# traveller59/spconv

Hardware: NVIDIA H100
Metric: active-voxels/sec fwd+bwd SubMConv3d 3^3 C=64 (higher is better)
Workload: dtype fp16

## Files before the change

### spconv_b200/csrc/common.cuh

```cuda
#pragma once
#include <cuda_runtime.h>
#include <cuda_fp16.h>
#include <cuda_bf16.h>
#include <stdint.h>
#include <stdio.h>
#include <string.h>
#include <stdarg.h>
#include <type_traits>

#include "../../include/spconv_b200.h"

namespace spx {

void set_error(const char *fmt, ...);
void count_launch(int n = 1);
void set_family(int f);
int sm_count();
int current_device();

struct RuntimeCfg {
    int force_simt = 0, force_tc = 0;
    bool tf32_dgrad_fma = false;
    bool tf32_wgrad_fma = false;
};
RuntimeCfg &runtime_cfg();

bool func_configured(const void *fn, int dev);

#define SPX_CHECK_CUDA(expr)                                                              \
    do {                                                                                  \
        cudaError_t _e = (expr);                                                          \
        if (_e != cudaSuccess) {                                                          \
            (void)cudaGetLastError();                                                     \
            spx::set_error("%s failed: %s (%s:%d)", #expr, cudaGetErrorString(_e),        \
                           __FILE__, __LINE__);                                           \
            return 1;                                                                     \
        }                                                                                 \
    } while (0)

#define SPX_CHECK_LAUNCH(name)                                                            \
    do {                                                                                  \
        cudaError_t _e = cudaGetLastError();                                              \
        if (_e != cudaSuccess) {                                                          \
            spx::set_error("launch of %s failed: %s (%s:%d)", name,                       \
                           cudaGetErrorString(_e), __FILE__, __LINE__);                   \
            return 1;                                                                     \
        }                                                                                 \
        spx::count_launch();                                                              \
    } while (0)

#define SPX_REQUIRE(cond, ...)                                                            \
    do {                                                                                  \
        if (!(cond)) {                                                                    \
            spx::set_error(__VA_ARGS__);                                                  \
            return 2;                                                                     \
        }                                                                                 \
    } while (0)

static inline size_t align_up(size_t x, size_t a) { return (x + a - 1) / a * a; }
static inline int64_t div_up64(int64_t a, int64_t b) { return (a + b - 1) / b; }

static inline bool aligned16(const void *p) { return ((uintptr_t)p & 15u) == 0; }

#define SPX_REQUIRE_ALIGNED16(ptr, who)                                                   \
    SPX_REQUIRE(spx::aligned16(ptr), "%s: %s must be 16-byte aligned (got %p)", who, #ptr, \
                (const void *)(ptr))

struct WorkspaceCarver {
    char *base;
    size_t off = 0, cap;
    WorkspaceCarver(void *p, size_t bytes) : base((char *)p), cap(bytes) {}
    template <typename T> T *take(size_t n) {
        off = align_up(off, 256);
        T *r = (T *)(base + off);
        off += n * sizeof(T);
        return r;
    }
    bool ok() const { return off <= cap; }
};

__host__ __device__ static inline int dtype_bytes(int dt) {
    switch (dt) {
        case SPX_F32: return 4;
        case SPX_F16: return 2;
        case SPX_BF16: return 2;
        case SPX_I8: return 1;
    }
    return 0;
}

#ifdef __CUDACC__

template <typename T> __device__ __forceinline__ float to_float(T v);
template <> __device__ __forceinline__ float to_float<float>(float v) { return v; }
template <> __device__ __forceinline__ float to_float<__half>(__half v) { return __half2float(v); }
template <> __device__ __forceinline__ float to_float<__nv_bfloat16>(__nv_bfloat16 v) { return __bfloat162float(v); }
template <> __device__ __forceinline__ float to_float<int8_t>(int8_t v) { return (float)v; }

template <typename T> __device__ __forceinline__ T from_float(float v);
template <> __device__ __forceinline__ float from_float<float>(float v) { return v; }
template <> __device__ __forceinline__ __half from_float<__half>(float v) { return __float2half_rn(v); }
template <> __device__ __forceinline__ __nv_bfloat16 from_float<__nv_bfloat16>(float v) { return __float2bfloat16_rn(v); }

__device__ __forceinline__ float apply_act(float v, int act, float alpha) {
    switch (act) {
        case SPX_ACT_RELU: return v > 0.f ? v : 0.f;
        case SPX_ACT_SIGMOID: return 1.f / (1.f + __expf(-v));
        case SPX_ACT_LEAKY_RELU: return v >= 0.f ? v : v * alpha;
        default: return v;
    }
}

__device__ __forceinline__ uint32_t smem_u32(const void *p) {
    return (uint32_t)__cvta_generic_to_shared(p);
}

__device__ __forceinline__ void mbar_init(uint64_t *bar, uint32_t count) {
    asm volatile("mbarrier.init.shared::cta.b64 [%0], %1;" ::"r"(smem_u32(bar)), "r"(count) : "memory");
}
__device__ __forceinline__ void mbar_fence_init() {
    asm volatile("fence.mbarrier_init.release.cluster;" ::: "memory");
}
__device__ __forceinline__ void mbar_arrive(uint64_t *bar) {
    asm volatile("{\n\t.reg .b64 st;\n\tmbarrier.arrive.shared::cta.b64 st, [%0];\n\t}" ::"r"(smem_u32(bar)) : "memory");
}
__device__ __forceinline__ void mbar_arrive_expect_tx(uint64_t *bar, uint32_t bytes) {
    asm volatile("{\n\t.reg .b64 st;\n\tmbarrier.arrive.expect_tx.shared::cta.b64 st, [%0], %1;\n\t}" ::"r"(smem_u32(bar)), "r"(bytes) : "memory");
}
__device__ __forceinline__ bool mbar_try_wait(uint64_t *bar, uint32_t parity) {
    uint32_t ok;
    asm volatile(
        "{\n\t.reg .pred p;\n\t"
        "mbarrier.try_wait.parity.shared::cta.b64 p, [%1], %2;\n\t"
        "selp.u32 %0, 1, 0, p;\n\t}"
        : "=r"(ok) : "r"(smem_u32(bar)), "r"(parity) : "memory");
    return ok != 0;
}
__device__ __forceinline__ void mbar_wait(uint64_t *bar, uint32_t parity) {
    if (mbar_try_wait(bar, parity)) return;
    const long long t0 = clock64();
    uint32_t spins = 0;
    while (!mbar_try_wait(bar, parity)) {
        if ((++spins & 0x3FFFu) == 0u && clock64() - t0 > 4000000000ll) {
            printf("spconv_b200: mbarrier wait timed out (block %d thread %d bar 0x%x parity %u)\n",
                   (int)blockIdx.x, (int)threadIdx.x, smem_u32(bar), parity);
            __trap();
        }
    }
}
__device__ __forceinline__ void mbar_wait_silent(uint64_t *bar, uint32_t parity) {
    if (mbar_try_wait(bar, parity)) return;
    const long long t0 = clock64();
    uint32_t spins = 0;
    while (!mbar_try_wait(bar, parity)) {
        if ((++spins & 0x3FFFu) == 0u && clock64() - t0 > 4000000000ll) __trap();
    }
}
__device__ __forceinline__ void cp_async_mbar_arrive_noinc(uint64_t *bar) {
    asm volatile("cp.async.mbarrier.arrive.noinc.shared::cta.b64 [%0];" ::"r"(smem_u32(bar)) : "memory");
}

__device__ __forceinline__ void cp_async_16(uint32_t dst_smem, const void *src, uint32_t src_bytes) {
    asm volatile("cp.async.cg.shared.global [%0], [%1], 16, %2;" ::"r"(dst_smem), "l"(src), "r"(src_bytes) : "memory");
}
__device__ __forceinline__ void cp_async_commit() { asm volatile("cp.async.commit_group;" ::: "memory"); }
template <int N> __device__ __forceinline__ void cp_async_wait() {
    asm volatile("cp.async.wait_group %0;" ::"n"(N) : "memory");
}

__device__ __forceinline__ void fence_proxy_async_smem() {
    asm volatile("fence.proxy.async.shared::cta;" ::: "memory");
}

__device__ __forceinline__ void tma_load_2d(uint32_t dst_smem, const void *tmap, uint64_t *bar,
                                            int32_t c0, int32_t c1) {
    asm volatile(
        "cp.async.bulk.tensor.2d.shared::cta.global.tile.mbarrier::complete_tx::bytes [%0], [%1, {%3, %4}], [%2];"
        ::"r"(dst_smem), "l"(tmap), "r"(smem_u32(bar)), "r"(c0), "r"(c1) : "memory");
}
__device__ __forceinline__ void bulk_copy_g2s(uint32_t dst_smem, const void *src, uint32_t bytes, uint64_t *bar) {
    asm volatile("cp.async.bulk.shared::cluster.global.mbarrier::complete_tx::bytes [%0], [%1], %2, [%3];"
                 ::"r"(dst_smem), "l"(src), "r"(bytes), "r"(smem_u32(bar)) : "memory");
}
__device__ __forceinline__ void tma_prefetch_desc(const void *tmap) {
    asm volatile("prefetch.tensormap [%0];" ::"l"(tmap) : "memory");
}

enum MmaKind { KIND_F16 = 0, KIND_TF32 = 1, KIND_I8 = 2 };

__device__ __forceinline__ void wgmma_fence() { asm volatile("wgmma.fence.sync.aligned;" ::: "memory"); }
__device__ __forceinline__ void wgmma_commit() { asm volatile("wgmma.commit_group.sync.aligned;" ::: "memory"); }
template <int N> __device__ __forceinline__ void wgmma_wait() {
    asm volatile("wgmma.wait_group.sync.aligned %0;" ::"n"(N) : "memory");
}
template <typename T, int R> __device__ __forceinline__ void fence_regs(T (&d)[R]) {
#pragma unroll
    for (int i = 0; i < R; ++i) {
        if constexpr (sizeof(T) == 4 && std::is_floating_point<T>::value) asm volatile("" : "+f"(d[i])::"memory");
        else asm volatile("" : "+r"(d[i])::"memory");
    }
}

__host__ __device__ __forceinline__ uint64_t gmma_desc_hi(uint32_t lbo_bytes, uint32_t sbo_bytes, uint32_t swizzle_bytes) {
    const uint64_t layout = swizzle_bytes == 128 ? 1ull : (swizzle_bytes == 64 ? 2ull : 3ull);
    return ((uint64_t)((lbo_bytes >> 4) & 0x3FFF) << 16) | ((uint64_t)((sbo_bytes >> 4) & 0x3FFF) << 32) | (layout << 62);
}

__device__ __forceinline__ uint32_t swizzle_offset(uint32_t off, uint32_t swizzle_bytes) {
    uint32_t bits = swizzle_bytes == 128 ? 7u : (swizzle_bytes == 64 ? 3u : 1u);
    return off ^ (((off >> 7) & bits) << 4);
}

#endif

}
```

### spconv_b200/csrc/gemm_tc.cu

```cuda
#include "gemm.cuh"
#include "wgmma.cuh"
#include <cuda.h>
#include <atomic>
#include <mutex>
#include <stdlib.h>

namespace spx {

constexpr int TC_TILE_M = 128;
constexpr int TC_CONS_WARPS = 8;
constexpr int TC_PROD_WARPS = 2;
constexpr int TC_PROD_THREADS = TC_PROD_WARPS * 32;
constexpr int TC_TMA_WARP = TC_CONS_WARPS + TC_PROD_WARPS;
constexpr int TC_SCHED_WARP = TC_TMA_WARP + 1;
constexpr int TC_THREADS = 3 * 128;
constexpr int TC_INFO_DEPTH = 4;
constexpr int TC_INFO_READERS = TC_PROD_WARPS + TC_CONS_WARPS + 1;
constexpr int TC_MAX_STAGES = 8;
constexpr int TC_SMEM_BUDGET = 200 * 1024;

struct TcParams {
    const uint8_t *x;
    int xb;
    int span_b, b_subtiles, b_sub_bytes, b_bytes, b_mn_major, b_kstep16_mn;
    int b_transposed;
    const float *w;
    int c_in, c_out;
    int w_inner_elems;
    int span_b_elems;
    int n;
    int ab_bf16;
    int stages, a_stage_bytes, stage_bytes, idx_bytes;
    int64_t rows;
    const int32_t *tile_table;
    const int32_t *sched_rec;
    int *sched_state;
    const int32_t *argsort;
    int kv, words, reverse;
    void *y;
    int out_dtype;
    int epi_mode;
    const void *bias;
    int act; float alpha;
    const float *scale, *bias_f32;
    const int8_t *output_add;
    float output_add_scale;
};

struct BitIter {
    uint32_t m0, m1, m2, m3;
    __device__ __forceinline__ BitIter(const uint32_t (&t)[4]) : m0(t[0]), m1(t[1]), m2(t[2]), m3(t[3]) {}
    __device__ __forceinline__ int next() {
        if (m0) { int b = __ffs(m0) - 1; m0 &= m0 - 1; return b; }
        if (m1) { int b = __ffs(m1) - 1; m1 &= m1 - 1; return 32 + b; }
        if (m2) { int b = __ffs(m2) - 1; m2 &= m2 - 1; return 64 + b; }
        if (m3) { int b = __ffs(m3) - 1; m3 &= m3 - 1; return 96 + b; }
        return -1;
    }
};

template <int OUT>
__device__ __forceinline__ void store2(uint8_t *dst, float a, float b) {
    if constexpr (OUT == SPX_F32) {
        *reinterpret_cast<float2 *>(dst) = make_float2(a, b);
    } else if constexpr (OUT == SPX_F16) {
        *reinterpret_cast<__half2 *>(dst) = __floats2half2_rn(a, b);
    } else if constexpr (OUT == SPX_BF16) {
        *reinterpret_cast<__nv_bfloat162 *>(dst) = __floats2bfloat162_rn(a, b);
    } else {
        const int qa = (int)fminf(fmaxf(rintf(a), -128.f), 127.f), qb = (int)fminf(fmaxf(rintf(b), -128.f), 127.f);
        *reinterpret_cast<uint16_t *>(dst) = (uint16_t)((uint32_t)(uint8_t)(int8_t)qa | ((uint32_t)(uint8_t)(int8_t)qb << 8));
    }
}

template <int OUT> struct OutElem { static constexpr int bytes = OUT == SPX_F32 ? 4 : (OUT == SPX_I8 ? 1 : 2); };

template <int OUT>
__device__ __forceinline__ float load_bias(const void *bias, int j) {
    if constexpr (OUT == SPX_F32) return ((const float *)bias)[j];
    else if constexpr (OUT == SPX_F16) return __half2float(((const __half *)bias)[j]);
    else return __bfloat162float(((const __nv_bfloat16 *)bias)[j]);
}

template <int OUT, bool INT8_MODE, int N, typename Acc, bool PLAIN = false>
__device__ __forceinline__ void epilogue_frag(const TcParams &p, const float *ec, const Acc (&acc)[N / 2], int64_t dst_lo,
                                              int64_t dst_hi, int lane) {
    if constexpr (!INT8_MODE && !PLAIN) {
        if (p.bias == nullptr && p.act == SPX_ACT_NONE) {
            epilogue_frag<OUT, false, N, Acc, true>(p, ec, acc, dst_lo, dst_hi, lane);
            return;
        }
    }
    constexpr int EB = OutElem<OUT>::bytes;
    const bool has_bias = !PLAIN && (INT8_MODE ? (p.bias_f32 != nullptr) : (p.bias != nullptr));
#pragma unroll
    for (int h = 0; h < 2; ++h) {
        const int64_t dst = h ? dst_hi : dst_lo;
        if (dst < 0) continue;
        uint8_t *row_ptr = (uint8_t *)p.y + dst * (int64_t)N * EB;
#pragma unroll
        for (int nb = 0; nb < N / 8; ++nb) {
            const int col = nb * 8 + 2 * (lane & 3);
            float f[2];
#pragma unroll
            for (int j = 0; j < 2; ++j) {
                const Acc v = acc[nb * 4 + 2 * h + j];
                if constexpr (!INT8_MODE) {
                    f[j] = (float)v;
                    if (has_bias) f[j] += ec[col + j];
                } else {
                    f[j] = (float)(int32_t)v * ec[col + j];
                    if (has_bias) f[j] += ec[N + col + j];
                    if (p.output_add) f[j] += (float)p.output_add[dst * (int64_t)N + col + j] * p.output_add_scale;
                }
                if (!PLAIN && p.act != SPX_ACT_NONE) f[j] = apply_act(f[j], p.act, p.alpha);
            }
            store2<OUT>(row_ptr + col * EB, f[0], f[1]);
        }
    }
}

template <int KIND, int N, typename Acc>
__device__ __forceinline__ void mma_step(Acc (&acc)[N / 2], uint64_t a, uint64_t b, int b_mn, int bf16) {
    if constexpr (KIND == KIND_F16) {
        if (bf16) {
            if (b_mn) Wgmma<N>::template bf16<0, 1>(acc, a, b, 1u);
            else Wgmma<N>::template bf16<0, 0>(acc, a, b, 1u);
        } else {
            if (b_mn) Wgmma<N>::template f16<0, 1>(acc, a, b, 1u);
            else Wgmma<N>::template f16<0, 0>(acc, a, b, 1u);
        }
    } else if constexpr (KIND == KIND_TF32) {
        Wgmma<N>::tf32(acc, a, b, 1u);
    } else {
        Wgmma<N>::s8(acc, a, b, 1u);
    }
}

template <int KIND, int CPR, int N>
__global__ void __launch_bounds__(TC_THREADS, 1)
tc_gather_gemm_kernel(const __grid_constant__ CUtensorMap tmap_w, const TcParams p) {
    using Acc = typename std::conditional<KIND == KIND_I8, int32_t, float>::type;
    constexpr int LG_CPR = CPR == 2 ? 1 : CPR == 4 ? 2 : CPR == 8 ? 3 : CPR == 16 ? 4 : 5;
    constexpr int RPI = 32 / CPR;
    constexpr int XB = CPR * 16;
    constexpr int SPAN_A = XB < 128 ? XB : 128;
    constexpr int LG_SPAN_A = SPAN_A == 128 ? 7 : (SPAN_A == 64 ? 6 : 5);
    constexpr int A_SUB_BYTES = TC_TILE_M * SPAN_A;
    constexpr int A_SUBTILES = XB / SPAN_A;
    constexpr int Q_A = SPAN_A / 32;
    constexpr int ROWS_PW = TC_TILE_M / TC_PROD_WARPS;
    constexpr int ITERS = ROWS_PW / RPI > 0 ? ROWS_PW / RPI : 1;
    static_assert(ROWS_PW * CPR >= 32, "a producer warp must cover at least one full cp.async instruction");

    extern __shared__ __align__(1024) uint8_t smem_raw[];
    const uint32_t raw_addr = smem_u32(smem_raw);
    const uint32_t pad = (1024u - (raw_addr & 1023u)) & 1023u;
    uint8_t *smem = smem_raw + pad;
    const uint32_t smem_base = raw_addr + pad;

    const uint32_t idx_off = (uint32_t)p.stages * p.stage_bytes;
    uint64_t *bars = reinterpret_cast<uint64_t *>(smem + idx_off + 2u * p.idx_bytes);
    uint64_t *full = bars;
    uint64_t *empty = bars + TC_MAX_STAGES;
    uint64_t *idx_full = bars + 2 * TC_MAX_STAGES;
    uint64_t *idx_empty = bars + 2 * TC_MAX_STAGES + 2;
    uint64_t *info_full = bars + 2 * TC_MAX_STAGES + 4;
    uint64_t *info_empty = bars + 2 * TC_MAX_STAGES + 4 + TC_INFO_DEPTH;
    int32_t *info = reinterpret_cast<int32_t *>(bars + 2 * TC_MAX_STAGES + 4 + 2 * TC_INFO_DEPTH);
    float *ec = reinterpret_cast<float *>(smem + idx_off + 2u * p.idx_bytes + 1024u);

    const int warp = threadIdx.x >> 5;
    const int lane = threadIdx.x & 31;
    const int64_t num_tiles = (p.rows + TC_TILE_M - 1) / TC_TILE_M;

    auto read_info = [&](int n, uint32_t (&tm)[4]) -> int {
        const int e = n & (TC_INFO_DEPTH - 1);
        mbar_wait_silent(&info_full[e], (uint32_t)((n / TC_INFO_DEPTH) & 1));
        const volatile int32_t *r = info + e * 8;
        const int tile = r[0];
        tm[0] = (uint32_t)r[1]; tm[1] = (uint32_t)r[2]; tm[2] = (uint32_t)r[3]; tm[3] = (uint32_t)r[4];
        __syncwarp();
        if (lane == 0) mbar_arrive(&info_empty[e]);
        return tile;
    };

    if (threadIdx.x == 0) {
        for (int s = 0; s < p.stages; ++s) {
            mbar_init(&full[s], TC_PROD_THREADS + 1);
            mbar_init(&empty[s], TC_CONS_WARPS);
        }
        for (int a = 0; a < 2; ++a) {
            mbar_init(&idx_full[a], 1);
            mbar_init(&idx_empty[a], TC_PROD_WARPS + TC_CONS_WARPS);
        }
        for (int e = 0; e < TC_INFO_DEPTH; ++e) {
            mbar_init(&info_full[e], 1);
            mbar_init(&info_empty[e], TC_INFO_READERS);
        }
        mbar_fence_init();
        tma_prefetch_desc(&tmap_w);
    }
    for (int j = threadIdx.x; j < N; j += TC_THREADS) {
        if constexpr (KIND == KIND_I8) {
            ec[j] = __ldg(p.scale + j);
            if (p.bias_f32) ec[N + j] = __ldg(p.bias_f32 + j);
        } else if (p.bias) {
            if constexpr (KIND == KIND_TF32) ec[j] = load_bias<SPX_F32>(p.bias, j);
            else ec[j] = p.out_dtype == SPX_F16 ? load_bias<SPX_F16>(p.bias, j) : load_bias<SPX_BF16>(p.bias, j);
        }
    }
    __syncthreads();

    if (warp >= TC_CONS_WARPS && warp < TC_TMA_WARP) {
        const int pw = warp - TC_CONS_WARPS;
        const int r0 = lane >> LG_CPR;
        const uint32_t byte_in_row = (uint32_t)(lane & (CPR - 1)) << 4;
        const uint8_t *x_lane = p.x + byte_in_row;
        uint32_t dst_off[ITERS];
#pragma unroll
        for (int itc = 0; itc < ITERS; ++itc) {
            const uint32_t row_in_tile = (uint32_t)(pw * ROWS_PW + r0 + itc * RPI);
            const uint32_t sub = byte_in_row >> LG_SPAN_A;
            const uint32_t within = byte_in_row & (uint32_t)(SPAN_A - 1);
            dst_off[itc] = sub * (uint32_t)A_SUB_BYTES + swizzle_offset((row_in_tile << LG_SPAN_A) + within, SPAN_A);
        }
        int stage = 0; uint32_t phase = 0;
        for (int n = 0;; ++n) {
            uint32_t tm[4];
            if (read_info(n, tm) < 0) break;
            const int buf = n & 1;
            mbar_wait_silent(&idx_full[buf], (uint32_t)((n >> 1) & 1));
            const int32_t *idx_lane = reinterpret_cast<const int32_t *>(smem + idx_off + (size_t)buf * p.idx_bytes) +
                                      pw * ROWS_PW + r0;
            BitIter it(tm);
            int k = it.next();
            int32_t ridx[ITERS];
            if (k >= 0) {
#pragma unroll
                for (int itc = 0; itc < ITERS; ++itc) ridx[itc] = idx_lane[k * 128 + itc * RPI];
            }
            while (k >= 0) {
                mbar_wait_silent(&empty[stage], phase ^ 1u);
                const uint32_t a_stage = smem_base + (uint32_t)stage * p.stage_bytes;
#pragma unroll
                for (int itc = 0; itc < ITERS; ++itc)
                    cp_async_16(a_stage + dst_off[itc], x_lane + (int64_t)max(ridx[itc], 0) * XB,
                                ridx[itc] >= 0 ? 16u : 0u);
                cp_async_mbar_arrive_noinc(&full[stage]);
                k = it.next();
                if (k >= 0) {
#pragma unroll
                    for (int itc = 0; itc < ITERS; ++itc) ridx[itc] = idx_lane[k * 128 + itc * RPI];
                }
                if (++stage == p.stages) { stage = 0; phase ^= 1u; }
            }
            __syncwarp();
            if (lane == 0) mbar_arrive(&idx_empty[buf]);
        }
    } else if (warp == TC_TMA_WARP) {
        int stage = 0; uint32_t phase = 0;
        for (int n = 0;; ++n) {
            uint32_t tm[4];
            if (read_info(n, tm) < 0) break;
            BitIter it(tm);
            for (int k = it.next(); k >= 0; k = it.next()) {
                mbar_wait_silent(&empty[stage], phase ^ 1u);
                const int kw = p.reverse ? p.kv - 1 - k : k;
                const uint32_t b_stage = smem_base + (uint32_t)stage * p.stage_bytes + p.a_stage_bytes;
                if (p.b_transposed) {
                    const int i4s = p.c_in >> 2;
                    const float *wk = p.w + (int64_t)kw * p.c_in;
                    for (int q = lane; q < p.c_out * i4s; q += 32) {
                        const int o = q / i4s, i4 = (q - o * i4s) * 4;
                        const float4 v = __ldg(reinterpret_cast<const float4 *>(wk + (int64_t)o * p.kv * p.c_in + i4));
                        const uint32_t kb = (uint32_t)o * 4u;
                        const uint32_t sub = kb / (uint32_t)p.span_b, within = kb % (uint32_t)p.span_b;
                        const float vv[4] = {v.x, v.y, v.z, v.w};
#pragma unroll
                        for (int t = 0; t < 4; ++t) {
                            const uint32_t off = sub * (uint32_t)p.b_sub_bytes +
                                                 swizzle_offset((uint32_t)(i4 + t) * (uint32_t)p.span_b + within, (uint32_t)p.span_b);
                            asm volatile("st.shared.f32 [%0], %1;" ::"r"(b_stage + off), "f"(vv[t]) : "memory");
                        }
                    }
                    fence_proxy_async_smem();
                    __syncwarp();
                    if (lane == 0) mbar_arrive(&full[stage]);
                } else if (lane == 0) {
                    mbar_arrive_expect_tx(&full[stage], (uint32_t)p.b_bytes);
                    for (int sb = 0; sb < p.b_subtiles; ++sb)
                        tma_load_2d(b_stage + sb * p.b_sub_bytes, &tmap_w, &full[stage],
                                    kw * p.w_inner_elems + sb * p.span_b_elems, 0);
                }
                __syncwarp();
                if (++stage == p.stages) { stage = 0; phase ^= 1u; }
            }
        }
    } else if (warp == TC_SCHED_WARP) {
        const uint32_t blk_bytes = (uint32_t)(p.kv + 1) * 512u;
        for (int n = 0;; ++n) {
            const int b = n & 1, e = n & (TC_INFO_DEPTH - 1);
            mbar_wait_silent(&idx_empty[b], (uint32_t)(((n >> 1) & 1) ^ 1));
            mbar_wait_silent(&info_empty[e], (uint32_t)(((n / TC_INFO_DEPTH) & 1) ^ 1));
            int tile = -1;
            if (lane == 0) {
                const int ticket = atomicAdd(p.sched_state, 1);
                int4 r0 = make_int4(-1, 1, 0, 0), r1 = make_int4(0, 0, 0, 0);
                if ((int64_t)ticket < num_tiles) {
                    const int4 *rp = reinterpret_cast<const int4 *>(p.sched_rec + (int64_t)ticket * TT_REC_INTS);
                    r0 = __ldg(rp); r1 = __ldg(rp + 1);
                }
                tile = r0.x;
                int32_t *dst = info + e * 8;
                dst[0] = r0.x; dst[1] = r0.y; dst[2] = r0.z; dst[3] = r0.w; dst[4] = r1.x;
                if (tile >= 0) {
                    mbar_arrive_expect_tx(&idx_full[b], blk_bytes);
                    bulk_copy_g2s(smem_base + idx_off + (uint32_t)b * p.idx_bytes,
                                  p.tile_table + (int64_t)tile * (p.kv + 1) * 128, blk_bytes, &idx_full[b]);
                }
                mbar_arrive(&info_full[e]);
            }
            tile = __shfl_sync(0xffffffffu, tile, 0);
            if (tile < 0) break;
        }
        if (lane == 0) {
            __threadfence();
            const int done = atomicAdd(p.sched_state + 1, 1);
            if (done == (int)gridDim.x - 1) {
                p.sched_state[0] = 0;
                p.sched_state[1] = 0;
                __threadfence();
            }
        }
        __syncwarp();
    } else if (warp < TC_CONS_WARPS) {
        const int wg = warp >> 2;
        int stage = 0; uint32_t phase = 0;
        const uint64_t a_hi = gmma_desc_hi(16u, 8u * SPAN_A, SPAN_A);
        const uint64_t b_hi = p.b_mn_major ? gmma_desc_hi((uint32_t)p.b_sub_bytes, 8u * p.span_b, p.span_b)
                                           : gmma_desc_hi(16u, 8u * p.span_b, p.span_b);
        const uint32_t b_sub16 = (uint32_t)p.b_sub_bytes >> 4;
        Acc acc[N / 2];
        for (int local = 0;; ++local) {
            uint32_t tm[4];
            const int tile = read_info(local, tm);
            if (tile < 0) break;
            int32_t d_lo, d_hi;
            {
                const int buf = local & 1;
                mbar_wait_silent(&idx_full[buf], (uint32_t)((local >> 1) & 1));
                const int32_t *dst = reinterpret_cast<const int32_t *>(smem + idx_off + (size_t)buf * p.idx_bytes) +
                                     p.kv * 128 + wg * 64 + (warp & 3) * 16 + (lane >> 2);
                d_lo = dst[0];
                d_hi = dst[8];
                __syncwarp();
                if (lane == 0) mbar_arrive(&idx_empty[buf]);
            }
#pragma unroll
            for (int i = 0; i < N / 2; ++i) acc[i] = (Acc)0;
            BitIter it(tm);
            int held = -1;
            for (int k = it.next(); k >= 0; k = it.next()) {
                mbar_wait_silent(&full[stage], phase);
                fence_proxy_async_smem();
                const uint32_t a16 = (smem_base + (uint32_t)stage * p.stage_bytes + (uint32_t)(wg * 64 * SPAN_A)) >> 4;
                const uint32_t b16 = (smem_base + (uint32_t)stage * p.stage_bytes + (uint32_t)p.a_stage_bytes) >> 4;
                fence_regs(acc);
                wgmma_fence();
                if (!p.b_mn_major) {
#pragma unroll
                    for (int sub = 0; sub < A_SUBTILES; ++sub) {
                        const uint32_t as = a16 + (uint32_t)sub * (uint32_t)(A_SUB_BYTES >> 4);
                        const uint32_t bs = b16 + (uint32_t)sub * b_sub16;
#pragma unroll
                        for (int jr = 0; jr < Q_A; ++jr)
                            mma_step<KIND, N>(acc, a_hi | (uint64_t)((as + 2u * jr) & 0x3FFFu),
                                              b_hi | (uint64_t)((bs + 2u * jr) & 0x3FFFu), 0, p.ab_bf16);
                    }
                } else {
#pragma unroll
                    for (int sub = 0; sub < A_SUBTILES; ++sub) {
                        const uint32_t as = a16 + (uint32_t)sub * (uint32_t)(A_SUB_BYTES >> 4);
#pragma unroll
                        for (int jr = 0; jr < Q_A; ++jr) {
                            const uint32_t j = (uint32_t)(sub * Q_A + jr);
                            mma_step<KIND, N>(acc, a_hi | (uint64_t)((as + 2u * jr) & 0x3FFFu),
                                              b_hi | (uint64_t)((b16 + j * (uint32_t)p.b_kstep16_mn) & 0x3FFFu), 1,
                                              p.ab_bf16);
                        }
                    }
                }
                wgmma_commit();
                wgmma_wait<1>();
                fence_regs(acc);
                if (held >= 0) {
                    __syncwarp();
                    if (lane == 0) mbar_arrive(&empty[held]);
                }
                held = stage;
                if (++stage == p.stages) { stage = 0; phase ^= 1u; }
            }
            wgmma_wait<0>();
            fence_regs(acc);
            if (held >= 0) {
                __syncwarp();
                if (lane == 0) mbar_arrive(&empty[held]);
            }
            if constexpr (KIND == KIND_F16) {
                if (p.out_dtype == SPX_F16) epilogue_frag<SPX_F16, false, N>(p, ec, acc, d_lo, d_hi, lane);
                else epilogue_frag<SPX_BF16, false, N>(p, ec, acc, d_lo, d_hi, lane);
            } else if constexpr (KIND == KIND_TF32) {
                epilogue_frag<SPX_F32, false, N>(p, ec, acc, d_lo, d_hi, lane);
            } else {
                if (p.out_dtype == SPX_I8) epilogue_frag<SPX_I8, true, N>(p, ec, acc, d_lo, d_hi, lane);
                else if (p.out_dtype == SPX_F32) epilogue_frag<SPX_F32, true, N>(p, ec, acc, d_lo, d_hi, lane);
                else epilogue_frag<SPX_F16, true, N>(p, ec, acc, d_lo, d_hi, lane);
            }
        }
    }

    __syncthreads();
}

typedef CUresult (*EncodeTiledFn)(CUtensorMap *, CUtensorMapDataType, cuuint32_t, void *, const cuuint64_t *,
                                  const cuuint64_t *, const cuuint32_t *, const cuuint32_t *, CUtensorMapInterleave,
                                  CUtensorMapSwizzle, CUtensorMapL2promotion, CUtensorMapFloatOOBfill);

static EncodeTiledFn get_encode_fn() {
    static EncodeTiledFn fn = nullptr;
    static std::once_flag once;
    std::call_once(once, [] {
        void *p = nullptr;
        cudaDriverEntryPointQueryResult q;
        if (cudaGetDriverEntryPoint("cuTensorMapEncodeTiled", &p, cudaEnableDefault, &q) == cudaSuccess &&
            q == cudaDriverEntryPointSuccess)
            fn = (EncodeTiledFn)p;
    });
    return fn;
}

int make_weight_tmap(CUtensorMap *tm, const void *w, int dtype, int kv, int c_in, int c_out, int span_bytes) {
    EncodeTiledFn fn = get_encode_fn();
    SPX_REQUIRE(fn != nullptr, "cuTensorMapEncodeTiled entry point not available (driver too old?)");
    const int e = dtype_bytes(dtype);
    CUtensorMapDataType dt = dtype == SPX_F16 ? CU_TENSOR_MAP_DATA_TYPE_FLOAT16
                           : dtype == SPX_BF16 ? CU_TENSOR_MAP_DATA_TYPE_BFLOAT16
                           : dtype == SPX_F32 ? CU_TENSOR_MAP_DATA_TYPE_FLOAT32
                                              : CU_TENSOR_MAP_DATA_TYPE_UINT8;
    cuuint64_t dims[2] = {(cuuint64_t)kv * c_in, (cuuint64_t)c_out};
    cuuint64_t strides[1] = {(cuuint64_t)kv * c_in * e};
    cuuint32_t box[2] = {(cuuint32_t)(span_bytes / e), (cuuint32_t)c_out};
    cuuint32_t estr[2] = {1, 1};
    CUtensorMapSwizzle sw = span_bytes == 128 ? CU_TENSOR_MAP_SWIZZLE_128B
                          : span_bytes == 64 ? CU_TENSOR_MAP_SWIZZLE_64B
                                             : CU_TENSOR_MAP_SWIZZLE_32B;
    CUresult r = fn(tm, dt, 2, const_cast<void *>(w), dims, strides, box, estr, CU_TENSOR_MAP_INTERLEAVE_NONE, sw,
                    CU_TENSOR_MAP_L2_PROMOTION_L2_256B, CU_TENSOR_MAP_FLOAT_OOB_FILL_NONE);
    SPX_REQUIRE(r == CUDA_SUCCESS, "cuTensorMapEncodeTiled failed with %d (kv=%d C=%d K=%d span=%d)", (int)r, kv, c_in,
                c_out, span_bytes);
    return 0;
}

static bool span_ok(int bytes) { return bytes == 32 || bytes == 64 || bytes == 128 || bytes == 256 || bytes == 512; }

static bool tc_shape_ok(int dtype, int kv, int c_in, int c_out, int transpose_w) {
    const int e = dtype_bytes(dtype);
    if (e == 0) return false;
    if (c_in > 256 || c_out > 256) return false;
    if (c_in % 16 || c_out % 16) return false;
    if (!span_ok(c_in * e) || !span_ok(c_out * e)) return false;
    const int cy = transpose_w ? c_in : c_out;
    if (cy % 16 || cy > 256) return false;
    const int xb = (transpose_w ? c_out : c_in) * e;
    if (dtype == SPX_I8 && (c_in % 32 || c_out % 32)) return false;
    size_t stage = align_up((size_t)TC_TILE_M * xb, 1024) + align_up((size_t)c_in * c_out * e, 1024);
    const size_t idx = align_up((size_t)(kv + 1) * 512, 1024);
    if (2 * idx + 2 * stage > (size_t)TC_SMEM_BUDGET) return false;
    return true;
}

static bool tc_operands_aligned(const GatherGemmArgs &a) { return aligned16(a.x) && aligned16(a.w) && aligned16(a.y); }

bool tc_gather_gemm_supported(const GatherGemmArgs &a) {
    if (a.dtype == SPX_I8) return false;
    if (!a.tile_table || !a.tile_mask) return false;
    if (!tc_operands_aligned(a)) return false;
    if (a.dtype == SPX_F32 && a.transpose_w && (runtime_cfg().tf32_dgrad_fma || (a.c_in * 4) % 128)) return false;
    if (((size_t)a.kv * a.c_in * dtype_bytes(a.dtype)) % 16) return false;
    return tc_shape_ok(a.dtype, a.kv, a.c_in, a.c_out, a.transpose_w);
}
bool tc_gather_gemm_int8_supported(const Int8Args &q) {
    if (!q.g.tile_table || !q.g.tile_mask) return false;
    if (!tc_operands_aligned(q.g)) return false;
    if (((size_t)q.g.kv * q.g.c_in) % 16) return false;
    return tc_shape_ok(SPX_I8, q.g.kv, q.g.c_in, q.g.c_out, 0);
}

static int fill_params(const GatherGemmArgs &a, TcParams &p) {
    memset(&p, 0, sizeof(p));
    const int e = dtype_bytes(a.dtype);
    const int cx = a.cx(), cy = a.cy();
    p.x = (const uint8_t *)a.x;
    p.xb = cx * e;
    const int span_a = p.xb < 128 ? p.xb : 128;
    const int wb = a.c_in * e;
    p.b_transposed = (a.dtype == SPX_F32 && a.transpose_w) ? 1 : 0;
    if (p.b_transposed) {
        p.span_b = span_a;
        p.b_subtiles = p.xb / span_a;
        p.b_sub_bytes = cy * span_a;
        p.b_mn_major = 0;
    } else {
        p.span_b = wb < 128 ? wb : 128;
        p.b_subtiles = wb / p.span_b;
        p.b_sub_bytes = a.c_out * p.span_b;
        p.b_mn_major = a.transpose_w;
    }
    p.b_bytes = a.c_out * wb;
    p.b_kstep16_mn = ((32 / e) * p.span_b) >> 4;
    p.w = (const float *)a.w;
    p.c_in = a.c_in; p.c_out = a.c_out;
    p.w_inner_elems = a.c_in;
    p.span_b_elems = p.span_b / e;
    p.n = cy;
    p.ab_bf16 = a.dtype == SPX_BF16;
    p.a_stage_bytes = (int)align_up((size_t)TC_TILE_M * p.xb, 1024);
    p.stage_bytes = p.a_stage_bytes + (int)align_up((size_t)p.b_bytes, 1024);
    p.idx_bytes = (int)align_up((size_t)(a.kv + 1) * 512, 1024);
    p.stages = (TC_SMEM_BUDGET - 2 * p.idx_bytes) / p.stage_bytes;
    if (p.stages > TC_MAX_STAGES) p.stages = TC_MAX_STAGES;
    SPX_REQUIRE(p.stages >= 2, "tc_gather_gemm: tile does not fit shared memory (stage %d bytes)", p.stage_bytes);
    p.rows = a.rows; p.tile_table = a.tile_table; p.argsort = a.argsort;
    {
        const int64_t tiles = div_up64(a.rows, TC_TILE_M);
        p.sched_rec = a.tile_table + tt_blocks_elems(tiles, a.kv);
        static std::atomic<unsigned> next_slot{0};
        const unsigned slot = next_slot.fetch_add(1, std::memory_order_relaxed) % (TT_STATE_INTS / 2);
        p.sched_state = const_cast<int *>(reinterpret_cast<const int *>(p.sched_rec + tiles * TT_REC_INTS)) + 2 * slot;
    }
    p.kv = a.kv; p.words = (a.kv + 31) / 32; p.reverse = a.reverse;
    p.y = a.y; p.out_dtype = a.dtype; p.epi_mode = 0; p.bias = a.bias; p.act = a.act; p.alpha = a.alpha;
    return 0;
}

template <int KIND, int CPR, int N>
static int launch_tc_n(const CUtensorMap &tm, const TcParams &p, cudaStream_t stream) {
    const size_t smem = (size_t)p.stages * p.stage_bytes + 2 * (size_t)p.idx_bytes + 1024  + 1024  +
                        2 * N * sizeof(float) ;
    if (!func_configured((const void *)tc_gather_gemm_kernel<KIND, CPR, N>, current_device())) {
        SPX_CHECK_CUDA(cudaFuncSetAttribute(tc_gather_gemm_kernel<KIND, CPR, N>, cudaFuncAttributeMaxDynamicSharedMemorySize,
                                            (int)(TC_SMEM_BUDGET + 2048 + 2 * N * sizeof(float))));
        SPX_CHECK_CUDA(cudaFuncSetAttribute(tc_gather_gemm_kernel<KIND, CPR, N>, cudaFuncAttributePreferredSharedMemoryCarveout, 100));
    }
    const int64_t tiles = div_up64(p.rows, TC_TILE_M);
    const int64_t max_ctas = (int64_t)sm_count();
    const int grid = (int)(tiles < max_ctas ? tiles : max_ctas);
    tc_gather_gemm_kernel<KIND, CPR, N><<<grid, TC_THREADS, smem, stream>>>(tm, p);
    SPX_CHECK_LAUNCH("tc_gather_gemm_kernel");
    return 0;
}

template <int KIND, int CPR>
static int launch_tc_cpr(const CUtensorMap &tm, const TcParams &p, cudaStream_t stream) {
    switch (p.n) {
        case 16: if constexpr (KIND != KIND_I8) return launch_tc_n<KIND, CPR, 16>(tm, p, stream); break;
        case 32: return launch_tc_n<KIND, CPR, 32>(tm, p, stream);
        case 64: return launch_tc_n<KIND, CPR, 64>(tm, p, stream);
        case 128: if constexpr (CPR != 32) return launch_tc_n<KIND, CPR, 128>(tm, p, stream); break;
        case 256: if constexpr (KIND != KIND_TF32 && CPR != 32) return launch_tc_n<KIND, CPR, 256>(tm, p, stream); break;
    }
    set_error("tc_gather_gemm: unsupported output channel count %d", p.n);
    return 2;
}

template <int KIND>
static int launch_tc(const CUtensorMap &tm, const TcParams &p, cudaStream_t stream) {
    switch (p.xb >> 4) {
        case 2: if constexpr (KIND != KIND_TF32) return launch_tc_cpr<KIND, 2>(tm, p, stream); break;
        case 4: return launch_tc_cpr<KIND, 4>(tm, p, stream);
        case 8: return launch_tc_cpr<KIND, 8>(tm, p, stream);
        case 16: return launch_tc_cpr<KIND, 16>(tm, p, stream);
        case 32: if constexpr (KIND != KIND_I8) return launch_tc_cpr<KIND, 32>(tm, p, stream); break;
    }
    set_error("tc_gather_gemm: unsupported row bytes %d", p.xb);
    return 2;
}

int tc_gather_gemm(const GatherGemmArgs &a, cudaStream_t stream) {
    TcParams p;
    if (fill_params(a, p)) return 2;
    CUtensorMap tm;
    if (make_weight_tmap(&tm, a.w, a.dtype, a.kv, a.c_in, a.c_out, p.b_transposed ? 128 : p.span_b)) return 2;
    if (a.dtype == SPX_F32) return launch_tc<KIND_TF32>(tm, p, stream);
    return launch_tc<KIND_F16>(tm, p, stream);
}

int tc_gather_gemm_int8(const Int8Args &q, cudaStream_t stream) {
    TcParams p;
    if (fill_params(q.g, p)) return 2;
    p.out_dtype = q.out_dtype;
    p.epi_mode = 1;
    p.scale = q.scale; p.bias_f32 = q.bias_f32; p.output_add = q.output_add;
    p.output_add_scale = q.output_add_scale;
    CUtensorMap tm;
    if (make_weight_tmap(&tm, q.g.w, SPX_I8, q.g.kv, q.g.c_in, q.g.c_out, p.span_b)) return 2;
    return launch_tc<KIND_I8>(tm, p, stream);
}

}
```

Before: 539.4 million.

## Stage epilogue through swizzled shared buffers and offload scattered stores to scheduler warp

Consumer warps now write the accumulator tile into a swizzled shared-memory output buffer using stmatrix, along with the destination row indices, and signal an mbarrier. The scheduler warp polls with non-blocking test_wait and performs coalesced 16-byte scattered row stores to global memory, overlapping output writeback with the next tile's MMA. Up to two output buffers are used, and the pipeline stage count may drop by one to fit shared memory. The risk is that one warp handles all the stores and the pipeline becomes shallower.

```diff
diff --git a/spconv_b200/csrc/common.cuh b/spconv_b200/csrc/common.cuh
--- a/spconv_b200/csrc/common.cuh
+++ b/spconv_b200/csrc/common.cuh
@@ -136,6 +136,15 @@
         : "=r"(ok) : "r"(smem_u32(bar)), "r"(parity) : "memory");
     return ok != 0;
 }
+__device__ __forceinline__ bool mbar_test_wait(uint64_t *bar, uint32_t parity) {
+    uint32_t ok;
+    asm volatile(
+        "{\n\t.reg .pred p;\n\t"
+        "mbarrier.test_wait.parity.shared::cta.b64 p, [%1], %2;\n\t"
+        "selp.u32 %0, 1, 0, p;\n\t}"
+        : "=r"(ok) : "r"(smem_u32(bar)), "r"(parity) : "memory");
+    return ok != 0;
+}
 __device__ __forceinline__ void mbar_wait(uint64_t *bar, uint32_t parity) {
     if (mbar_try_wait(bar, parity)) return;
     const long long t0 = clock64();
diff --git a/spconv_b200/csrc/gemm_tc.cu b/spconv_b200/csrc/gemm_tc.cu
--- a/spconv_b200/csrc/gemm_tc.cu
+++ b/spconv_b200/csrc/gemm_tc.cu
@@ -18,6 +18,9 @@
 constexpr int TC_INFO_READERS = TC_PROD_WARPS + TC_CONS_WARPS + 1;
 constexpr int TC_MAX_STAGES = 8;
 constexpr int TC_SMEM_BUDGET = 200 * 1024;
+constexpr int TC_SMEM_LIMIT = 227 * 1024;
+constexpr int TC_EC_BYTES = 2 * 256 * 4;
+constexpr int TC_MAX_OUT_BUFS = 2;
 
 struct TcParams {
     const uint8_t *x;
@@ -45,6 +48,7 @@
     const float *scale, *bias_f32;
     const int8_t *output_add;
     float output_add_scale;
+    int out_bufs, out_bytes, out_row_bytes, out_row_lg;
 };
 
 struct BitIter {
@@ -60,20 +64,49 @@
 };
 
 template <int OUT>
-__device__ __forceinline__ void store2(uint8_t *dst, float a, float b) {
-    if constexpr (OUT == SPX_F32) {
-        *reinterpret_cast<float2 *>(dst) = make_float2(a, b);
-    } else if constexpr (OUT == SPX_F16) {
-        *reinterpret_cast<__half2 *>(dst) = __floats2half2_rn(a, b);
+__device__ __forceinline__ uint32_t pack2(float a, float b) {
+    if constexpr (OUT == SPX_F16) {
+        const __half2 h = __floats2half2_rn(a, b);
+        return *reinterpret_cast<const uint32_t *>(&h);
     } else if constexpr (OUT == SPX_BF16) {
-        *reinterpret_cast<__nv_bfloat162 *>(dst) = __floats2bfloat162_rn(a, b);
+        const __nv_bfloat162 h = __floats2bfloat162_rn(a, b);
+        return *reinterpret_cast<const uint32_t *>(&h);
     } else {
         const int qa = (int)fminf(fmaxf(rintf(a), -128.f), 127.f), qb = (int)fminf(fmaxf(rintf(b), -128.f), 127.f);
-        *reinterpret_cast<uint16_t *>(dst) = (uint16_t)((uint32_t)(uint8_t)(int8_t)qa | ((uint32_t)(uint8_t)(int8_t)qb << 8));
-    }
+        return (uint32_t)(uint8_t)(int8_t)qa | ((uint32_t)(uint8_t)(int8_t)qb << 8);
+    }
+}
+
+template <int OUT>
+__device__ __forceinline__ void store2(uint8_t *dst, float a, float b) {
+    if constexpr (OUT == SPX_F32) *reinterpret_cast<float2 *>(dst) = make_float2(a, b);
+    else if constexpr (OUT == SPX_I8) *reinterpret_cast<uint16_t *>(dst) = (uint16_t)pack2<OUT>(a, b);
+    else *reinterpret_cast<uint32_t *>(dst) = pack2<OUT>(a, b);
 }
 
 template <int OUT> struct OutElem { static constexpr int bytes = OUT == SPX_F32 ? 4 : (OUT == SPX_I8 ? 1 : 2); };
+
+template <bool INT8_MODE, bool PLAIN, int N, typename Acc>
+__device__ __forceinline__ float epi_value(const TcParams &p, const float *ec, Acc v, bool has_bias, int64_t dst, int col) {
+    float f;
+    if constexpr (!INT8_MODE) {
+        f = (float)v;
+        if (has_bias) f += ec[col];
+    } else {
+        f = (float)(int32_t)v * ec[col];
+        if (has_bias) f += ec[N + col];
+        if (p.output_add && dst >= 0) f += (float)p.output_add[dst * (int64_t)N + col] * p.output_add_scale;
+    }
+    if (!PLAIN && p.act != SPX_ACT_NONE) f = apply_act(f, p.act, p.alpha);
+    return f;
+}
+
+__device__ __forceinline__ uint32_t out_swz(uint32_t off) { return off ^ (((off >> 7) & 7u) << 4); }
+
+__device__ __forceinline__ void stmatrix_x4(uint32_t addr, uint32_t r0, uint32_t r1, uint32_t r2, uint32_t r3) {
+    asm volatile("stmatrix.sync.aligned.m8n8.x4.shared.b16 [%0], {%1, %2, %3, %4};" ::"r"(addr), "r"(r0), "r"(r1),
+                 "r"(r2), "r"(r3) : "memory");
+}
 
 template <int OUT>
 __device__ __forceinline__ float load_bias(const void *bias, int j) {
@@ -101,21 +134,76 @@
 #pragma unroll
         for (int nb = 0; nb < N / 8; ++nb) {
             const int col = nb * 8 + 2 * (lane & 3);
-            float f[2];
-#pragma unroll
-            for (int j = 0; j < 2; ++j) {
-                const Acc v = acc[nb * 4 + 2 * h + j];
-                if constexpr (!INT8_MODE) {
-                    f[j] = (float)v;
-                    if (has_bias) f[j] += ec[col + j];
-                } else {
-                    f[j] = (float)(int32_t)v * ec[col + j];
-                    if (has_bias) f[j] += ec[N + col + j];
-                    if (p.output_add) f[j] += (float)p.output_add[dst * (int64_t)N + col + j] * p.output_add_scale;
-                }
-                if (!PLAIN && p.act != SPX_ACT_NONE) f[j] = apply_act(f[j], p.act, p.alpha);
-            }
-            store2<OUT>(row_ptr + col * EB, f[0], f[1]);
+            const float f0 = epi_value<INT8_MODE, PLAIN, N>(p, ec, acc[nb * 4 + 2 * h], has_bias, dst, col);
+            const float f1 = epi_value<INT8_MODE, PLAIN, N>(p, ec, acc[nb * 4 + 2 * h + 1], has_bias, dst, col + 1);
+            store2<OUT>(row_ptr + col * EB, f0, f1);
+        }
+    }
+}
+
+template <int OUT, int N, typename Acc, bool PLAIN = false>
+__device__ __forceinline__ void epilogue_stage(const TcParams &p, const float *ec, const Acc (&acc)[N / 2], int64_t dst_lo,
+                                               int64_t dst_hi, uint32_t tile_s, int wrow, int lane) {
+    if constexpr (!PLAIN) {
+        if (p.bias == nullptr && p.act == SPX_ACT_NONE) {
+            epilogue_stage<OUT, N, Acc, true>(p, ec, acc, dst_lo, dst_hi, tile_s, wrow, lane);
+            return;
+        }
+    }
+    constexpr int EB = OutElem<OUT>::bytes;
+    constexpr uint32_t RB = (uint32_t)N * EB;
+    const bool has_bias = !PLAIN && p.bias != nullptr;
+    if constexpr (EB == 2) {
+        const uint32_t arow = (uint32_t)(wrow + ((lane >> 3) & 1) * 8 + (lane & 7));
+#pragma unroll
+        for (int nb = 0; nb < N / 8; nb += 2) {
+            uint32_t r[4];
+#pragma unroll
+            for (int q = 0; q < 4; ++q) {
+                const int h = q & 1, b = nb + (q >> 1), col = b * 8 + 2 * (lane & 3);
+                const int64_t dst = h ? dst_hi : dst_lo;
+                r[q] = pack2<OUT>(epi_value<false, PLAIN, N>(p, ec, acc[b * 4 + 2 * h], has_bias, dst, col),
+                                  epi_value<false, PLAIN, N>(p, ec, acc[b * 4 + 2 * h + 1], has_bias, dst, col + 1));
+            }
+            stmatrix_x4(tile_s + out_swz(arow * RB + (uint32_t)(nb + (lane >> 4)) * 16u), r[0], r[1], r[2], r[3]);
+        }
+    } else {
+#pragma unroll
+        for (int h = 0; h < 2; ++h) {
+            const int64_t dst = h ? dst_hi : dst_lo;
+            const uint32_t row_off = (uint32_t)(wrow + h * 8 + (lane >> 2)) * RB;
+#pragma unroll
+            for (int nb = 0; nb < N / 8; ++nb) {
+                const int col = nb * 8 + 2 * (lane & 3);
+                const float f0 = epi_value<false, PLAIN, N>(p, ec, acc[nb * 4 + 2 * h], has_bias, dst, col);
+                const float f1 = epi_value<false, PLAIN, N>(p, ec, acc[nb * 4 + 2 * h + 1], has_bias, dst, col + 1);
+                asm volatile("st.shared.v2.f32 [%0], {%1, %2};" ::"r"(tile_s + out_swz(row_off + (uint32_t)col * EB)),
+                             "f"(f0), "f"(f1) : "memory");
+            }
+        }
+    }
+}
+
+__device__ __forceinline__ void store_staged_tile(const TcParams &p, const uint8_t *buf, uint32_t buf_s, int lane) {
+    const uint32_t rb = (uint32_t)p.out_row_bytes;
+    const int lg = p.out_row_lg;
+    const int32_t *d = reinterpret_cast<const int32_t *>(buf + TC_TILE_M * rb);
+    const int chunks = TC_TILE_M << lg;
+    for (int q0 = 0; q0 < chunks; q0 += 128) {
+        uint4 v[4];
+        int64_t dst[4];
+#pragma unroll
+        for (int u = 0; u < 4; ++u) {
+            const uint32_t q = (uint32_t)(q0 + u * 32 + lane);
+            dst[u] = d[q >> lg];
+            asm volatile("ld.shared.v4.u32 {%0, %1, %2, %3}, [%4];"
+                         : "=r"(v[u].x), "=r"(v[u].y), "=r"(v[u].z), "=r"(v[u].w) : "r"(buf_s + out_swz(q * 16u)));
+        }
+#pragma unroll
+        for (int u = 0; u < 4; ++u) {
+            const uint32_t q = (uint32_t)(q0 + u * 32 + lane);
+            if (dst[u] >= 0)
+                *reinterpret_cast<uint4 *>((uint8_t *)p.y + dst[u] * (int64_t)rb + ((q & ((1u << lg) - 1u)) << 4)) = v[u];
         }
     }
 }
@@ -168,7 +256,12 @@
     uint64_t *info_full = bars + 2 * TC_MAX_STAGES + 4;
     uint64_t *info_empty = bars + 2 * TC_MAX_STAGES + 4 + TC_INFO_DEPTH;
     int32_t *info = reinterpret_cast<int32_t *>(bars + 2 * TC_MAX_STAGES + 4 + 2 * TC_INFO_DEPTH);
+    uint64_t *out_full = reinterpret_cast<uint64_t *>(info + TC_INFO_DEPTH * 8);
+    uint64_t *out_empty = out_full + TC_MAX_OUT_BUFS;
     float *ec = reinterpret_cast<float *>(smem + idx_off + 2u * p.idx_bytes + 1024u);
+    const uint32_t out_off = idx_off + 2u * p.idx_bytes + 1024u + (uint32_t)TC_EC_BYTES;
+    constexpr bool STAGED_OK = N <= 128 && KIND != KIND_I8;
+    const int out_bufs = STAGED_OK ? p.out_bufs : 0;
 
     const int warp = threadIdx.x >> 5;
     const int lane = threadIdx.x & 31;
@@ -197,6 +290,10 @@
         for (int e = 0; e < TC_INFO_DEPTH; ++e) {
             mbar_init(&info_full[e], 1);
             mbar_init(&info_empty[e], TC_INFO_READERS);
+        }
+        for (int b = 0; b < TC_MAX_OUT_BUFS; ++b) {
+            mbar_init(&out_full[b], TC_CONS_WARPS);
+            mbar_init(&out_empty[b], 1);
         }
         mbar_fence_init();
         tma_prefetch_desc(&tmap_w);
@@ -299,10 +396,48 @@
         }
     } else if (warp == TC_SCHED_WARP) {
         const uint32_t blk_bytes = (uint32_t)(p.kv + 1) * 512u;
-        for (int n = 0;; ++n) {
+        int n = 0;
+        int m = 0;
+        int ob = 0;
+        uint32_t oph = 0;
+        int end = -1;
+        long long t0 = 0;
+        uint32_t idle = 0;
+        for (;;) {
             const int b = n & 1, e = n & (TC_INFO_DEPTH - 1);
-            mbar_wait_silent(&idx_empty[b], (uint32_t)(((n >> 1) & 1) ^ 1));
-            mbar_wait_silent(&info_empty[e], (uint32_t)(((n / TC_INFO_DEPTH) & 1) ^ 1));
+            int work = 0;
+            if (lane == 0) {
+                if (end < 0 && out_bufs == 0) {
+                    mbar_wait_silent(&idx_empty[b], (uint32_t)(((n >> 1) & 1) ^ 1));
+                    mbar_wait_silent(&info_empty[e], (uint32_t)(((n / TC_INFO_DEPTH) & 1) ^ 1));
+                    work = 1;
+                } else if (end < 0 && mbar_test_wait(&idx_empty[b], (uint32_t)(((n >> 1) & 1) ^ 1)) &&
+                           mbar_test_wait(&info_empty[e], (uint32_t)(((n / TC_INFO_DEPTH) & 1) ^ 1)))
+                    work = 1;
+                else if (out_bufs && m < (end < 0 ? n : end) &&
+                         mbar_test_wait(&out_full[ob], oph))
+                    work = 2;
+                else if (end >= 0 && (out_bufs == 0 || m == end))
+                    work = 3;
+            }
+            work = __shfl_sync(0xffffffffu, work, 0);
+            if (work == 3) break;
+            if (work == 0) {
+                if (idle++ == 0) t0 = clock64();
+                else if ((idle & 0x3FFFu) == 0u && clock64() - t0 > 4000000000ll) __trap();
+                continue;
+            }
+            idle = 0;
+            if (work == 2) {
+                mbar_wait_silent(&out_full[ob], oph);
+                store_staged_tile(p, smem + out_off + (uint32_t)ob * p.out_bytes, smem_base + out_off + (uint32_t)ob * p.out_bytes,
+                                  lane);
+                __syncwarp();
+                if (lane == 0) mbar_arrive(&out_empty[ob]);
+                ++m;
+                if (++ob == out_bufs) { ob = 0; oph ^= 1u; }
+                continue;
+            }
             int tile = -1;
             if (lane == 0) {
                 const int ticket = atomicAdd(p.sched_state, 1);
@@ -322,7 +457,8 @@
                 mbar_arrive(&info_full[e]);
             }
             tile = __shfl_sync(0xffffffffu, tile, 0);
-            if (tile < 0) break;
+            if (tile < 0) end = n;
+            ++n;
         }
         if (lane == 0) {
             __threadfence();
@@ -341,6 +477,7 @@
         const uint64_t b_hi = p.b_mn_major ? gmma_desc_hi((uint32_t)p.b_sub_bytes, 8u * p.span_b, p.span_b)
                                            : gmma_desc_hi(16u, 8u * p.span_b, p.span_b);
         const uint32_t b_sub16 = (uint32_t)p.b_sub_bytes >> 4;
+        int ob = 0; uint32_t oph = 0;
         Acc acc[N / 2];
         for (int local = 0;; ++local) {
             uint32_t tm[4];
@@ -406,6 +543,29 @@
             if (held >= 0) {
                 __syncwarp();
                 if (lane == 0) mbar_arrive(&empty[held]);
+            }
+            if (out_bufs) {
+                if constexpr (STAGED_OK) {
+                    mbar_wait_silent(&out_empty[ob], oph ^ 1u);
+                    const uint32_t tile_s = smem_base + out_off + (uint32_t)ob * p.out_bytes;
+                    const int wrow = wg * 64 + (warp & 3) * 16;
+                    if ((lane & 3) == 0) {
+                        int32_t *d = reinterpret_cast<int32_t *>(smem + out_off + (uint32_t)ob * p.out_bytes +
+                                                                 TC_TILE_M * (uint32_t)p.out_row_bytes);
+                        d[wrow + (lane >> 2)] = d_lo;
+                        d[wrow + 8 + (lane >> 2)] = d_hi;
+                    }
+                    if constexpr (KIND == KIND_F16) {
+                        if (p.out_dtype == SPX_F16) epilogue_stage<SPX_F16, N>(p, ec, acc, d_lo, d_hi, tile_s, wrow, lane);
+                        else epilogue_stage<SPX_BF16, N>(p, ec, acc, d_lo, d_hi, tile_s, wrow, lane);
+                    } else {
+                        epilogue_stage<SPX_F32, N>(p, ec, acc, d_lo, d_hi, tile_s, wrow, lane);
+                    }
+                    __syncwarp();
+                    if (lane == 0) mbar_arrive(&out_full[ob]);
+                    if (++ob == out_bufs) { ob = 0; oph ^= 1u; }
+                }
+                continue;
             }
             if constexpr (KIND == KIND_F16) {
                 if (p.out_dtype == SPX_F16) epilogue_frag<SPX_F16, false, N>(p, ec, acc, d_lo, d_hi, lane);
@@ -544,13 +704,31 @@
     return 0;
 }
 
+static void plan_epilogue(TcParams &p) {
+    p.out_row_bytes = p.n * dtype_bytes(p.out_dtype);
+    p.out_row_lg = __builtin_ctz((unsigned)p.out_row_bytes >> 4);
+    p.out_bytes = (int)align_up((size_t)TC_TILE_M * (p.out_row_bytes + 4), 1024);
+    p.out_bufs = 0;
+    if (p.n > 128 || p.epi_mode == 1) return;
+    const int fixed = 2 * p.idx_bytes + 1024  + 1024  + TC_EC_BYTES;
+    for (int nb = TC_MAX_OUT_BUFS; nb >= 1; --nb) {
+        const int fit = (TC_SMEM_LIMIT - fixed - nb * p.out_bytes) / p.stage_bytes;
+        const int s = fit < p.stages ? fit : p.stages;
+        if (s >= 2 && s >= p.stages - 1) {
+            p.stages = s;
+            p.out_bufs = nb;
+            return;
+        }
+    }
+}
+
 template <int KIND, int CPR, int N>
 static int launch_tc_n(const CUtensorMap &tm, const TcParams &p, cudaStream_t stream) {
     const size_t smem = (size_t)p.stages * p.stage_bytes + 2 * (size_t)p.idx_bytes + 1024  + 1024  +
-                        2 * N * sizeof(float) ;
+                        TC_EC_BYTES  + (size_t)p.out_bufs * p.out_bytes ;
     if (!func_configured((const void *)tc_gather_gemm_kernel<KIND, CPR, N>, current_device())) {
         SPX_CHECK_CUDA(cudaFuncSetAttribute(tc_gather_gemm_kernel<KIND, CPR, N>, cudaFuncAttributeMaxDynamicSharedMemorySize,
-                                            (int)(TC_SMEM_BUDGET + 2048 + 2 * N * sizeof(float))));
+                                            TC_SMEM_LIMIT));
         SPX_CHECK_CUDA(cudaFuncSetAttribute(tc_gather_gemm_kernel<KIND, CPR, N>, cudaFuncAttributePreferredSharedMemoryCarveout, 100));
     }
     const int64_t tiles = div_up64(p.rows, TC_TILE_M);
@@ -590,6 +768,7 @@
 int tc_gather_gemm(const GatherGemmArgs &a, cudaStream_t stream) {
     TcParams p;
     if (fill_params(a, p)) return 2;
+    plan_epilogue(p);
     CUtensorMap tm;
     if (make_weight_tmap(&tm, a.w, a.dtype, a.kv, a.c_in, a.c_out, p.b_transposed ? 128 : p.span_b)) return 2;
     if (a.dtype == SPX_F32) return launch_tc<KIND_TF32>(tm, p, stream);
@@ -603,6 +782,7 @@
     p.epi_mode = 1;
     p.scale = q.scale; p.bias_f32 = q.bias_f32; p.output_add = q.output_add;
     p.output_add_scale = q.output_add_scale;
+    plan_epilogue(p);
     CUtensorMap tm;
     if (make_weight_tmap(&tm, q.g.w, SPX_I8, q.g.kv, q.g.c_in, q.g.c_out, p.span_b)) return 2;
     return launch_tc<KIND_I8>(tm, p, stream);
```

Result: no change. 544.7 million, median of 6 (+1.0%).
